# TUM-DAML/gemnet_pytorch

Hardware: AMD Instinct MI355X
Metric: molecules/sec (forward+force) GemNet-T on COLL-shaped batches (higher is better)
Workload: dtype f32

## Files before the change

gemnet_pytorch_amd/csrc/radial_head.hip:

```cpp
#include "common.h"
#include "basis_math.h"

namespace {

constexpr int RH_NR = 6, RH_S = 7, RH_NI = 16;
constexpr int RH_NFUN = RH_NR + RH_S * RH_NR;
constexpr int RH_NOUT = 3 + RH_S;

constexpr int RH_LPE = 16, RH_BLOCK = 256, RH_EPB = RH_BLOCK / RH_LPE;

__device__ __forceinline__ float rh_distance(const float* __restrict__ R, int c, int a, float& vx, float& vy, float& vz) {
  const float* Ra = R + 3 * (int64_t)a;
  const float* Rc = R + 3 * (int64_t)c;
  vx = Ra[0] - Rc[0]; vy = Ra[1] - Rc[1]; vz = Ra[2] - Rc[2];
  return sqrtf(vx * vx + vy * vy + vz * vz);
}

__global__ void __launch_bounds__(RH_BLOCK)
radial_head_fwd_kernel(const float* __restrict__ R, const int32_t* __restrict__ id_c, const int32_t* __restrict__ id_a,
                       const float* __restrict__ freq, const float* __restrict__ z, const double* __restrict__ nrm,
                       const float* __restrict__ wcat, float* __restrict__ rbf, float* __restrict__ rbf3,
                       float* __restrict__ rbf_h, float* __restrict__ rbf_out, float* __restrict__ rbf_W1, int64_t E,
                       double cutoff, int p) {
  __shared__ float vals[RH_EPB][RH_NFUN];
// ... 53 lines not shown
  const int64_t e = blockIdx.x * (int64_t)RH_EPB + el;
  const bool ok = e < E;
  float vx = 0.f, vy = 0.f, vz = 0.f, d = 1.f;
  double g = 0.0;
  if (ok) {
    d = rh_distance(R, id_c[e], id_a[e], vx, vy, vz);
    const bool any_rbf = g_rbf || g_rbf3 || g_rbf_h || g_rbf_out;
    for (int j = sub; j < RH_NFUN; j += RH_LPE) {
      if (j < RH_NR) {
        if (!any_rbf) continue;
        float c = g_rbf ? g_rbf[e * RH_NR + j] : 0.f;
        if (g_rbf3) c += rh_dot16(wcat + (0 * RH_NR + j) * RH_NI, g_rbf3 + e * RH_NI);
        if (g_rbf_h) c += rh_dot16(wcat + (1 * RH_NR + j) * RH_NI, g_rbf_h + e * RH_NI);
        if (g_rbf_out) c += rh_dot16(wcat + (2 * RH_NR + j) * RH_NI, g_rbf_out + e * RH_NI);
        g += (double)c * bessel_rbf_eval((double)d, (double)freq[j], cutoff, p, 1, 0);
      } else if (g_rbf_W1) {
        const int lr = j - RH_NR, s = lr / RH_NR;
        const float c = rh_dot16(wcat + (3 * RH_NR + lr) * RH_NI, g_rbf_W1 + (e * RH_S + s) * RH_NI);
        g += (double)c * sph_radial_eval((double)d, (double)z[lr], nrm[lr], s, cutoff, p, 1);
      }
    }
  }
  part[el][sub] = g;
  __syncthreads();
  if (ok && sub == 0) {
    double t = 0.0;
#pragma unroll
    for (int q = 0; q < RH_LPE; ++q) t += part[el][q];
    const float sc = (float)(t / (double)d);
    Wout[3 * e] = sc * vx; Wout[3 * e + 1] = sc * vy; Wout[3 * e + 2] = sc * vz;
  }
}

inline bool rh_aligned(const void* p) { return (reinterpret_cast<uintptr_t>(p) & 15u) == 0; }

inline bool rh_shape_ok(int64_t E, int NR, int S, int NI, int p) {
  return NR == RH_NR && S == RH_S && NI == RH_NI && p >= 2 && E < ((int64_t)1 << 34);
}

}

extern "C" int gn_radial_head_fwd_f32(const float* R, const int32_t* id_c, const int32_t* id_a, const float* freq,
                                      const float* z, const double* nrm, const float* wcat, float* rbf, float* rbf3,
                                      float* rbf_h, float* rbf_out, float* rbf_W1, int64_t E, int NR, int S, int NI,
                                      float cutoff, int p, void* stream) {
  if (E <= 0) return 0;
  if (!rh_shape_ok(E, NR, S, NI, p)) return (int)hipErrorInvalidValue;
  if (!R || !id_c || !id_a || !freq || !z || !nrm || !wcat || !rbf || !rbf3 || !rbf_h || !rbf_out || !rbf_W1)
    return (int)hipErrorInvalidValue;
  hipLaunchKernelGGL(radial_head_fwd_kernel, dim3((unsigned)((E + RH_EPB - 1) / RH_EPB)), dim3(RH_BLOCK), 0,
                     static_cast<hipStream_t>(stream), R, id_c, id_a, freq, z, nrm, wcat, rbf, rbf3, rbf_h, rbf_out, rbf_W1, E,
                     (double)cutoff, p);
  GN_LAUNCH_CHECK();
  return 0;
}

extern "C" int gn_radial_head_bwd_f32(const float* g_rbf, const float* g_rbf3, const float* g_rbf_h, const float* g_rbf_out,
                                      const float* g_rbf_W1, const float* R, const int32_t* id_c, const int32_t* id_a,
                                      const float* freq, const float* z, const double* nrm, const float* wcat, float* W,
                                      int64_t E, int NR, int S, int NI, float cutoff, int p, void* stream) {
  if (E <= 0) return 0;
  if (!rh_shape_ok(E, NR, S, NI, p)) return (int)hipErrorInvalidValue;
  if (!R || !id_c || !id_a || !freq || !z || !nrm || !wcat || !W) return (int)hipErrorInvalidValue;
  if (!rh_aligned(wcat) || !rh_aligned(g_rbf3) || !rh_aligned(g_rbf_h) || !rh_aligned(g_rbf_out) || !rh_aligned(g_rbf_W1))
    return (int)hipErrorInvalidValue;
  hipLaunchKernelGGL(radial_head_bwd_kernel, dim3((unsigned)((E + RH_EPB - 1) / RH_EPB)), dim3(RH_BLOCK), 0,
                     static_cast<hipStream_t>(stream), g_rbf, g_rbf3, g_rbf_h, g_rbf_out, g_rbf_W1, R, id_c, id_a, freq, z, nrm, wcat,
                     W, E, (double)cutoff, p);
  GN_LAUNCH_CHECK();
  return 0;
}
```

gemnet_pytorch_amd/kernels.py:

```python
import contextlib
import ctypes
import os
import threading

import torch

from . import _lib
from ._lib import (GN_ANG_F16, GN_CHAIN_MAX_OPS, GN_CHAIN_ROW, GN_SPLIT_F16X2_ROW, GemmArgs, addr, check, ptr,
                   require_device, stream)


def _f32c(t):
    if t.dtype != torch.float32:
        raise TypeError(f"HIP path is fp32; got {t.dtype}")
    return t.contiguous()


def _rowmajor(t):
    if t.dtype != torch.float32:
        raise TypeError(f"HIP path is fp32; got {t.dtype}")
    if t.dim() != 2:
        raise ValueError("2-D operand expected")
    if t.shape[0] > 0 and t.shape[1] > 0 and t.stride(1) == 1 and t.stride(0) >= t.shape[1]:
        return t
# ... 601 lines not shown
    if idx_c.shape != idx_a.shape or idx_c.dim() != 1 or idx_c.dtype != torch.int32 or idx_a.dtype != torch.int32:
        raise ValueError("radial head: id_c / id_a are (E,) int32")
    return _f32c(R), idx_c.contiguous(), idx_a.contiguous(), _f32c(freq), _f32c(z), nrm.contiguous(), _f32c(wcat)


def radial_head_fwd(R, idx_c, idx_a, freq, z, nrm, wcat, cutoff, p):
    R, idx_c, idx_a, freq, z, nrm, wcat = _radial_head_args(R, idx_c, idx_a, freq, z, nrm, wcat)
    E = idx_c.shape[0]
    NR, S, NI = RADIAL_HEAD_SHAPE
    new = lambda *shape: torch.empty(shape, device=R.device, dtype=torch.float32)
    rbf, rbf3, rbf_h, rbf_out, rbf_W1 = new(E, NR), new(E, NI), new(E, NI), new(E, NI), new(E, S, NI)
    check(_lib.load().gn_radial_head_fwd_f32(ptr(R), ptr(idx_c), ptr(idx_a), ptr(freq), ptr(z), ptr(nrm), ptr(wcat), ptr(rbf),
                                             ptr(rbf3), ptr(rbf_h), ptr(rbf_out), ptr(rbf_W1), E, NR, S, NI, cutoff, p,
                                             stream()), "gn_radial_head_fwd_f32")
    return rbf, rbf3, rbf_h, rbf_out, rbf_W1


def radial_head_bwd(g_rbf, g_rbf3, g_rbf_h, g_rbf_out, g_rbf_W1, R, idx_c, idx_a, freq, z, nrm, wcat, cutoff, p):
    R, idx_c, idx_a, freq, z, nrm, wcat = _radial_head_args(R, idx_c, idx_a, freq, z, nrm, wcat)
    E = idx_c.shape[0]
    NR, S, NI = RADIAL_HEAD_SHAPE
    gs = []
    for g, shape in ((g_rbf, (E, NR)), (g_rbf3, (E, NI)), (g_rbf_h, (E, NI)), (g_rbf_out, (E, NI)), (g_rbf_W1, (E, S, NI))):
        if g is not None:
            require_device(g)
            if tuple(g.shape) != shape:
                raise ValueError(f"radial head: cotangent of shape {tuple(g.shape)}, expected {shape}")
            g = _f32c(g)
        gs.append(g)
    W = torch.empty((E, 3), device=R.device, dtype=torch.float32)
    check(_lib.load().gn_radial_head_bwd_f32(*[ptr(g) for g in gs], ptr(R), ptr(idx_c), ptr(idx_a), ptr(freq), ptr(z), ptr(nrm),
                                             ptr(wcat), ptr(W), E, NR, S, NI, cutoff, p, stream()),
          "gn_radial_head_bwd_f32")
    return W


def trip_basis_fwd(R, tc, ta, tb, S, want_theta=False):
    require_device(R, tc, ta, tb)
    R = _f32c(R)
    T = tc.shape[0]
    Y = torch.empty((T, S), device=R.device, dtype=torch.float32)
    theta = torch.empty(T, device=R.device, dtype=torch.float32) if want_theta else None
    check(_lib.load().gn_trip_basis_fwd_f32(ptr(R), ptr(tc), ptr(ta), ptr(tb), ptr(Y), ptr(theta), T, S, stream()),
          "gn_trip_basis_fwd_f32")
    return Y, theta


def trip_basis_bwd(gY, R, tc, ta, tb):
    require_device(gY, R)
    gY, R = _f32c(gY), _f32c(R)
    T, S = gY.shape
    Gc = torch.empty((T, 3), device=R.device, dtype=torch.float32)
    Gb = torch.empty((T, 3), device=R.device, dtype=torch.float32)
    check(_lib.load().gn_trip_basis_bwd_f32(ptr(gY), ptr(R), ptr(tc), ptr(ta), ptr(tb), ptr(Gc), ptr(Gb), T, S,
                                            stream()), "gn_trip_basis_bwd_f32")
    return Gc, Gb


def dist_fwd(R, id_c, id_a):
    require_device(R, id_c, id_a)
    R = _f32c(R)
    D = torch.empty(id_c.shape[0], device=R.device, dtype=torch.float32)
    check(_lib.load().gn_dist_fwd_f32(ptr(R), ptr(id_c), ptr(id_a), ptr(D), id_c.shape[0], stream()), "gn_dist_fwd_f32")
    return D


# ... 933 lines not shown
```

gemnet_pytorch_amd/model/gemnet.py:

```python
import contextlib
import os

import torch

from .. import ops
from ..graph import GraphPlan
from .layers import (INV_SQRT_2, AtomEmbedding, BesselBasisLayer, Dense, EdgeEmbedding,
                     EfficientInteractionDownProjection, InteractionBlock,
                     InteractionBlockTripletsOnly, OutputBlock, SphericalBasisLayer, TensorBasisLayer)
from .scaling import AutomaticFit


_nullcontext = contextlib.nullcontext
_H3_GUARD = os.environ.get("GEMNET_H3_GUARD", "1") == "1"
_TRAIN_OVERLAP = os.environ.get("GEMNET_TRAIN_OVERLAP", "1") == "1"
_Q_OVERLAP = os.environ.get("GEMNET_Q_OVERLAP", "1") == "1"
_RBF_OUT_SIDE = os.environ.get("GEMNET_RBF_OUT_SIDE", "1") == "1"
_PLAN_LATE = os.environ.get("GEMNET_PLAN_LATE", "1") == "1"


def K_chain_mode():
    from .. import kernels
    return kernels.current_mode()

# ... 123 lines not shown

    @staticmethod
    def calculate_angles(R, plan):
        q = plan.quad_geom
        Ra = ops.gather_rows(R, q["a_of_exp"])
        Rb = ops.gather_rows(R, q["b_of_exp"])
        Rd = ops.gather_rows(R, q["d_of_exp"])
        R_ba, R_bd = Ra - Rb, Rd - Rb
        angle_abd = GemNet.calculate_neighbor_angles(R_ba, R_bd)
        R_bd_proj = ops.gather_rows(GemNet.vector_rejection(R_bd, R_ba), plan.quad.expand)

        Rc = ops.gather_rows(R, q["c_of_red"])
        Ra2 = ops.gather_rows(R, q["a_of_red"])
        Rb2 = ops.gather_rows(R, q["b_of_red"])
        R_ac, R_ab = Rc - Ra2, Rb2 - Ra2
        angle_cab = ops.gather_rows(GemNet.calculate_neighbor_angles(R_ab, R_ac)[:, None], q["reduce_cab"])[:, 0]
        R_ac_proj = ops.gather_rows(GemNet.vector_rejection(R_ac, R_ab), q["reduce_cab"])
        angle_cabd = GemNet.calculate_neighbor_angles(R_ac_proj, R_bd_proj)
        return angle_cab, angle_abd, angle_cabd

    def _energy(self, R, plan, V=None, force_terms=False, Vint=None):
        T = self.triplets_only
        b3 = self.cbf_basis3
        overlap = self.overlap_output_blocks and (not ops.train2_enabled() or _TRAIN_OVERLAP)
        side = self._side_stream(R.device) if overlap and R.is_cuda and (T or _Q_OVERLAP) else None
        fork = side is not None and ops.is_fused() and T
        main = torch.cuda.current_stream(R.device) if fork else None
        h = terms = rbf_W1_3 = rbf_h = rbf_out = None
        proj = (self.mlp_rbf3, self.mlp_rbf_h, self.mlp_rbf_out)
        head = (ops.is_fused() and T and V is None and not self.direct_forces and R.is_cuda
                and all(d.bias is None and not d.act for d in proj)
                and ops.radial_head_supported(tuple(d.weight for d in proj) + (self.mlp_cbf3.weight,), b3.z_ln,
                                              self.rbf_basis.frequencies))
        if ops.is_fused():
            if fork:
                side.wait_stream(main)
                with torch.cuda.stream(side):
                    sph3 = ops.share_gradient(self._trip_basis3(R, plan, V))
                    h = self.atom_emb(plan.z_rows)
                    terms = self.edge_emb.atom_terms(h)
                    ev_a = torch.cuda.Event()
                    ev_a.record(side)
            if V is not None:
                from .. import pbc
                D_ca, rbf, rad3 = pbc.edge_basis(V, self.rbf_basis.frequencies, b3.z_ln, b3.n_ln, b3.cutoff, b3.p)
                V_ca = None
            elif head:
                rbf, rbf3, rbf_h, rbf_out, rbf_W1_3 = self._radial_head(R, plan, proj)
                V_ca = None
            else:
                D_ca, V_ca, rbf, rad3 = ops.edge_basis(R, self.rbf_basis.frequencies, plan.id_c, plan.id_a,
                                                       b3.z_ln, b3.n_ln, b3.cutoff, b3.p,
                                                       want_V=self.direct_forces)
            if fork and head:
                main.wait_event(ev_a)
                for t in (sph3, h) + tuple(terms):
                    t.record_stream(main)
            elif fork:
                ev_1 = torch.cuda.Event()
                ev_1.record(main)
                side.wait_event(ev_1)
                with torch.cuda.stream(side):
                    rbf.record_stream(side)
                    rad3.record_stream(side)
                    rbf_W1_3 = self.mlp_cbf3(rad3)
                    rbf_h = self.mlp_rbf_h(rbf)
                    if _RBF_OUT_SIDE:
                        rbf_out = self.mlp_rbf_out(rbf)
                    ev_b = torch.cuda.Event()
                    ev_b.record(side)
                if not _RBF_OUT_SIDE:
                    rbf_out = self.mlp_rbf_out(rbf)
                main.wait_event(ev_a)
                for t in (sph3, h) + tuple(terms):
                    t.record_stream(main)
            else:
                sph3 = ops.share_gradient(self._trip_basis3(R, plan, V))
        elif ops.train2_enabled() and not self.direct_forces:
            from .. import ops_train
            if V is not None:
                D_ca, V_ca = ops_train.distances_vec(V), None
                angles = ops_train.triplet_angles_vec(V, plan.trip)
            else:
                D_ca, V_ca = ops_train.distances(R, plan.id_c, plan.id_a), None
                angles = ops_train.triplet_angles(R, plan.t_c, plan.t_a, plan.t_b)
            rbf = self.rbf_basis(D_ca)
            rad3, sph3 = b3(D_ca, angles)
        elif V is not None:
            D_ca, V_ca = torch.sqrt(torch.sum(V ** 2, dim=1)), None
# ... 20 lines not shown
            if self.mlp_cbf4.bias is None and not self.mlp_cbf4.act:
                cbf4 = ops.cbf_project(rad4, plan.intm_ab, y_abd, self.mlp_cbf4.weight)
            cbf4_done = cbf4 is not None
            if not cbf4_done:
                cbf4 = (ops.gather_rows(rad4, plan.intm_ab) * y_abd[:, :, None]).reshape(-1, S * NR)
            ang = self.int_blocks[0].quad_interaction.mlp_sbf.weight.shape[:2] == (32, 32)
            if V is not None:
                sbf4 = (rad3, ops.share_gradient(pbc.quad_basis(V, Vint, plan, S, angle_form=ang)))
            else:
                sbf4 = (rad3, ops.share_gradient(ops.quad_basis(R, plan.q_c, plan.q_a, plan.q_b, plan.q_d, S, plan=plan,
                                                                angle_form=ang)))
        elif not T:
            qi = self.int_blocks[0].quad_interaction.mlp_sbf.weight
            if (ops.train2_enabled() and not self.direct_forces and self.num_spherical == 7
                    and ops.quad_train2_enabled(qi.shape[0], qi.shape[1], self.num_spherical ** 2)):
                from .. import ops_train
                qg = plan.quad_geom
                D_ab = ops_train.distances(R, plan.int_b, plan.int_a)
                Phi_abd = ops_train.triplet_angles(R, qg["a_of_exp"], qg["b_of_exp"], qg["d_of_exp"])
                cbf4 = self.cbf_basis(D_ab, Phi_abd, plan.intm_ab)
                sbf4 = (rad3, ops_train.quad_angles(R, plan.q_c, plan.q_a, plan.q_b, plan.q_d, plan))
            else:
                if ops.train2_enabled() and not self.direct_forces:
                    from .. import ops_train
                    D_ab = ops_train.distances(R, plan.int_b, plan.int_a)
                else:
                    D_ab, _ = self.calculate_interatomic_vectors(R, plan.int_b, plan.int_a)
                Phi_cab, Phi_abd, Theta_cabd = self.calculate_angles(R, plan)
                cbf4 = self.cbf_basis(D_ab, Phi_abd, plan.intm_ab)
                sbf4 = (rad3, ops.ylm(Phi_cab, Theta_cabd, self.num_spherical))

        if h is None:
            h = self.atom_emb(plan.z_rows)
        rbf = ops.accumulate_gradient(rbf)
        m = self.edge_emb(h, rbf, plan.id_c, plan.id_a, terms=terms)

        if not T:
            rbf4 = ops.accumulate_gradient(self.mlp_rbf4(rbf))
            if not cbf4_done:
                cbf4 = self.mlp_cbf4(cbf4)
            cbf4 = ops.accumulate_gradient(cbf4)
            sbf4 = (ops.accumulate_gradient(self.mlp_sbf4(sbf4[0])), sbf4[1])
        else:
            rbf4 = cbf4 = sbf4 = None
        rbf3 = ops.accumulate_gradient(rbf3 if head else self.mlp_rbf3(rbf))
        if head:
            cbf3 = (ops.accumulate_gradient(rbf_W1_3), sph3)
            rbf_h = ops.accumulate_gradient(rbf_h)
        elif fork:
            main.wait_event(ev_b)
            for t in (rbf_W1_3, rbf_h):
                t.record_stream(main)
            cbf3 = (ops.accumulate_gradient(rbf_W1_3, stream=main), sph3)
            rbf_h = ops.accumulate_gradient(rbf_h, stream=main)
        else:
            cbf3 = (ops.accumulate_gradient(self.mlp_cbf3(rad3)), sph3)
            rbf_h = ops.accumulate_gradient(self.mlp_rbf_h(rbf))
            rbf_out = self.mlp_rbf_out(rbf)

        outs = []
        group = self._out_group_blocks(R, m, rbf_out)
        group_ms = []

        def ready():
            if side is None:
                return None
            ev = torch.cuda.Event()
            ev.record(torch.cuda.current_stream())
# ... 30 lines not shown
        else:
            E_a, F_ca = outs[-1][0], outs[0][1]
            if force_terms:
                F_ca = [F for _, F in outs]
                if side is not None:
                    for F in F_ca:
                        F.record_stream(torch.cuda.current_stream())
            else:
                for _, F in outs[1:]:
                    F_ca = F_ca + F

        E_mol = ops.segsum_rows(E_a, plan.batch_seg)
        if not self.extensive:
            E_mol = E_mol / plan.atoms_per_mol.clamp(min=1)[:, None]
        return E_mol, F_ca, V_ca

    def _out_group_blocks(self, R, m, rbf_out):
        if not (self.triplets_only and R.is_cuda and ops.is_fused() and ops.constant_weights() and not ops.train2_enabled()
                and not self.direct_forces and not AutomaticFit.fitting_mode and ops.USE_OUT_GROUP):
            return None
        blocks = []
        for ob in self.out_blocks:
            if not (ob.fuse_aggregate and not ob.direct_forces and ob.dense_rbf.bias is None and not ob.dense_rbf.act
                    and ob._stackable(ob.seq_energy) and ob.out_energy.bias is None and not ob.out_energy.act
                    and ob.out_energy.weight.shape[0] == 1):
                return None
            gemms = [ob.seq_energy[0].weight]
            for layer in ob.seq_energy[1:]:
                gemms += [layer.dense_mlp[0].weight, layer.dense_mlp[1].weight]
            blocks.append(dict(W_rbf=ob.dense_rbf.weight, scale=ob.scale_sum.scale_factor, gemms=gemms,
                               act0=bool(ob.seq_energy[0].act), w_out=ob.out_energy.weight))
        return blocks if ops.output_group_supported(blocks, [m] * len(blocks), rbf_out) else None

    def _radial_head(self, R, plan, proj):
        b3 = self.cbf_basis3
        return ops.radial_head(R, self.rbf_basis.frequencies, plan.id_c, plan.id_a, b3.z_ln, b3.n_ln,
                               tuple(d.weight for d in proj) + (self.mlp_cbf3.weight,), b3.cutoff, b3.p)

    def _trip_basis3(self, R, plan, V):
        if V is not None:
            from .. import pbc
            return pbc.trip_basis(V, plan.trip, self.num_spherical)
        return ops.trip_basis(R, plan.t_c, plan.t_a, plan.t_b, self.num_spherical)

    def forward(self, inputs, stress=False):
        periodic = inputs.get("cell") is not None
        if stress and not periodic:
            raise ValueError("stress=True needs a periodic batch (inputs['cell'])")
        if periodic and "cell_offsets" not in inputs:
            raise ValueError("a periodic batch needs its neighbour list with 'cell_offsets' (pbc.PeriodicGraphBuilder)")
        inputs = self.with_indices(inputs)
        with ops.exclusive():
            out = self._forward_guarded(inputs, stress)
        return out if (stress or not periodic) else out[:2]

    def with_indices(self, inputs):
        if "id_c" in inputs:
            return inputs
        from ..index_device import ensure_indices
        self._check_inputs(inputs["R"])
        if torch.cuda.is_current_stream_capturing():
            raise RuntimeError("inputs without index arrays inside a stream capture: call model.with_indices(inputs) first")
        cutoff, int_cutoff = self.cbf_basis3.cutoff, getattr(getattr(self, "cbf_basis", None), "cutoff", 10.0)
        if "cutoffs" in inputs:
            c = inputs["cutoffs"].detach().cpu().tolist()
            cutoff, int_cutoff = float(c[0]), float(c[1])
        return ensure_indices(inputs, cutoff, int_cutoff, self.triplets_only)

# ... 327 lines not shown
```

gemnet_pytorch_amd/ops.py:

```python
import contextlib

import os
import threading

import torch

from . import _lib
from . import kernels as K

_EXCLUSIVE = threading.RLock()


def exclusive():
    return _EXCLUSIVE


_PARAM_GRADS = True


@contextlib.contextmanager
def param_grads(enabled: bool):
    global _PARAM_GRADS
    old = _PARAM_GRADS
    _PARAM_GRADS = enabled
# ... 809 lines not shown
            and all(W.is_cuda and W.dtype == torch.float32 for W in weights))


def _radial_head_wcat(weights):
    key = ("rhead",) + tuple((W.data_ptr(), tuple(W.stride())) for W in weights)
    return _cached(key, tuple(W._version for W in weights), lambda: K.radial_head_weights(*[W.detach() for W in weights]))


class _RadialHead(torch.autograd.Function):

    @staticmethod
    def forward(ctx, R, freq, ri_c, ri_a, z, nrm, wcat, cutoff, p):
        outs = K.radial_head_fwd(R, ri_c.idx32, ri_a.idx32, freq, z, nrm, wcat, cutoff, p)
        ctx.save_for_backward(R, freq, z, nrm, wcat)
        ctx.cfg = (ri_c, ri_a, cutoff, p)
        ctx.set_materialize_grads(False)
        return outs

    @staticmethod
    @torch.autograd.function.once_differentiable
    def backward(ctx, g_rbf, g_rbf3, g_rbf_h, g_rbf_out, g_rbf_W1):
        R, freq, z, nrm, wcat = ctx.saved_tensors
        ri_c, ri_a, cutoff, p = ctx.cfg
        gR = None
        if ctx.needs_input_grad[0]:
            W = K.radial_head_bwd(g_rbf, g_rbf3, g_rbf_h, g_rbf_out, g_rbf_W1, R, ri_c.idx32, ri_a.idx32, freq, z, nrm, wcat,
                                  cutoff, p)
            gR = K.segsum_multi([(W, *ri_a.csr, 1.0), (W, *ri_c.csr, -1.0)], ri_a.n_rows)
        return gR, None, None, None, None, None, None, None, None


def radial_head(R, freq, ri_c, ri_a, z, nrm, weights, cutoff, p):
    return _RadialHead.apply(R, freq.detach(), ri_c, ri_a, z, nrm, _radial_head_wcat(weights), float(cutoff), int(p))


class _TripBasis(torch.autograd.Function):

    @staticmethod
    def forward(ctx, R, ri_c, ri_a, ri_b, S):
        Y, _ = K.trip_basis_fwd(R, ri_c.idx32, ri_a.idx32, ri_b.idx32, S)
        ctx.save_for_backward(R)
        ctx.cfg = (ri_c, ri_a, ri_b)
        return Y

    @staticmethod
    @torch.autograd.function.once_differentiable
    def backward(ctx, gY):
        (R,) = ctx.saved_tensors
        ri_c, ri_a, ri_b = ctx.cfg
        if not ctx.needs_input_grad[0]:
            return None, None, None, None, None
        Gc, Gb = K.trip_basis_bwd(gY, R, ri_c.idx32, ri_a.idx32, ri_b.idx32)
        gR = K.segsum_multi([(Gc, *ri_c.csr, 1.0), (Gb, *ri_b.csr, 1.0), (Gc, *ri_a.csr, -1.0), (Gb, *ri_a.csr, -1.0)],
                            ri_c.n_rows)
        return gR, None, None, None, None


def trip_basis(R, ri_c, ri_a, ri_b, S):
    return _TripBasis.apply(R, ri_c, ri_a, ri_b, int(S))


def constant_weights():
    return _FUSED and not _PARAM_GRADS


USE_STACKS = os.environ.get("GEMNET_STACKS", "1") == "1"
# ... 736 lines not shown
```

include/gemnet_hip.h:

```cpp
#ifndef GEMNET_HIP_H
#define GEMNET_HIP_H

#include <stdint.h>

#ifdef __cplusplus
extern "C" {
#endif

int gn_abi_version(void);
const char* gn_error_string(int code);

typedef struct {
  const float* A; const float* B; float* C;
  int M, N, K;
  int lda, ldb, ldc;
  int trans_a, trans_b;
  const float* a_dact_pre;
  int act;
  float* pre_out;
  const float* mul; int ldmul;
  float alpha;
  const float* res; int ldres;
  float beta;
  const float* gadd1; const int32_t* gidx1;
// ... 215 lines not shown
                         float* dSm, int64_t E, int S, int C, int I, int O, float alpha, int accumulate, void* stream);
int gn_bil_up_bwd_f32(const float* G, const int32_t* inv_swap, const float* z_ac, const float* z_ca, const void* Wupt_planes,
                      const void* W2_planes, const float* Sm, const float* B, float* gB, float* dSm, int64_t E, int S, int C, int I,
                      int O, int N_up, float alpha, float alpha_up, int act, int accumulate, void* stream);
int gn_bil_dy_multi_f32(const float* const* dSm_list, const float* const* x_list, int nb, const int32_t* expand_idx,
                        const int32_t* seg_off, float* dY, int64_t E, int S, int C, void* stream);
int gn_bil_dy_atoms_f32(const float* const* dSm_list, const float* const* x_list, int nb, const int32_t* grp_rows,
                        const int32_t* grp_off, const int32_t* ent_off, const int32_t* ent_t, const int32_t* ent_bc,
                        const int32_t* expand_idx, const int32_t* seg_off, float* dY, int64_t G, int max_rows, int S, int C,
                        void* stream);

int gn_bessel_rbf_f32(const float* d, const float* freq, float* out, int64_t E, int R,
                      float cutoff, int p, int kd, int kf, void* stream);
int gn_sph_radial_f32(const float* d, const float* z, const double* nrm, float* out, int64_t E,
                      int S, int R, float cutoff, int p, int kd, void* stream);
int gn_ylm0_f32(const float* theta, float* out, int64_t T, int S, int k, void* stream);
int gn_ylm_f32(const float* theta, const float* phi, float* out, int64_t Q, int S, int kt, int kp,
               void* stream);

int gn_edge_basis_fwd_f32(const float* R, const int32_t* id_c, const int32_t* id_a, const float* freq,
                          const float* z, const double* nrm, float* D, float* V, float* rbf, float* rad,
                          int64_t E, int NR, int S, float cutoff, int p, void* stream);
int gn_edge_basis_bwd_f32(const float* g_D, const float* g_rbf, const float* g_rad, const float* R,
                          const int32_t* id_c, const int32_t* id_a, const float* freq, const float* z,
                          const double* nrm, float* W, int64_t E, int NR, int S, float cutoff, int p,
                          void* stream);
int gn_radial_head_fwd_f32(const float* R, const int32_t* id_c, const int32_t* id_a, const float* freq, const float* z,
                           const double* nrm, const float* wcat, float* rbf, float* rbf3, float* rbf_h, float* rbf_out,
                           float* rbf_W1, int64_t E, int NR, int S, int NI, float cutoff, int p, void* stream);
int gn_radial_head_bwd_f32(const float* g_rbf, const float* g_rbf3, const float* g_rbf_h, const float* g_rbf_out,
                           const float* g_rbf_W1, const float* R, const int32_t* id_c, const int32_t* id_a,
                           const float* freq, const float* z, const double* nrm, const float* wcat, float* W, int64_t E,
                           int NR, int S, int NI, float cutoff, int p, void* stream);
int gn_trip_basis_fwd_f32(const float* R, const int32_t* tc, const int32_t* ta, const int32_t* tb, float* Y,
                          float* theta, int64_t T, int S, void* stream);
int gn_trip_basis_bwd_f32(const float* gY, const float* R, const int32_t* tc, const int32_t* ta,
                          const int32_t* tb, float* Gc, float* Gb, int64_t T, int S, void* stream);

int gn_dist_fwd_f32(const float* R, const int32_t* id_c, const int32_t* id_a, float* D, int64_t E, void* stream);
int gn_dist_bwd_f32(const float* gD, const float* R, const int32_t* id_c, const int32_t* id_a, float* W, int64_t E, void* stream);
int gn_dist_jvp_f32(const float* R, const float* tR, const float* gD, const int32_t* id_c, const int32_t* id_a, float* Ddot,
                    float* H, int64_t E, void* stream);
int gn_angle_fwd_f32(const float* R, const int32_t* tc, const int32_t* ta, const int32_t* tb, float* theta, int64_t T,
                     void* stream);
int gn_angle_bwd_f32(const float* g, const float* R, const int32_t* tc, const int32_t* ta, const int32_t* tb, float* Gc,
                     float* Gb, int64_t T, void* stream);
int gn_angle_jvp_f32(const float* R, const float* tR, const float* g, const int32_t* tc, const int32_t* ta, const int32_t* tb,
                     float* thdot, float* Hc, float* Hb, int64_t T, void* stream);

int gn_quad_basis_fwd_f32(const float* R, const int32_t* qc, const int32_t* qa, const int32_t* qb,
                          const int32_t* qd, float* Y, int64_t Q, int S, void* stream);
int gn_quad_basis_bwd_f32(const float* gY, const float* R, const int32_t* qc, const int32_t* qa,
                          const int32_t* qb, const int32_t* qd, float* Gc, float* Gb, float* Gd, int64_t Q,
                          int S, void* stream);
int gn_quad_basis_bwd_ld_f32(const float* gY, const float* R, const int32_t* qc, const int32_t* qa, const int32_t* qb,
                             const int32_t* qd, float* Gc, int ldc, float* Gb, int ldb, float* Gd, int ldd, int64_t Q,
                             int S, void* stream);

int gn_ssilu_f32(const float* x, float* out, int64_t n, int k, void* stream);
int gn_pm_f32(const float* z, int k, const float* a, const float* b, const float* d, float c, float* out,
              int64_t n, void* stream);
int gn_dact_mul_f32(const float* g, const float* z, int act, const float* mul, float c, float* dz,
                    float* gmul, int64_t n, void* stream);

int gn_optim_blocks(int64_t n);
int gn_adamw_ema_step_f32(float* p, const float* g, const float* gscale, const float* wd, float* m, float* v,
// ... 95 lines not shown
```

Baseline: 16860.

## Fuse edge embedding into radial head kernel using per-element atom term tables

Adds forward and backward radial-head kernels that also compute the edge embedding m = ssilu(T_c[z_c] + T_a[z_a] + rbf·W_r). They use precomputed per-element tables (embedding times weight slices), cached across calls by weight version. This removes the separate rbf materialisation, the atom-term gather and the dense GEMM over edges. The backward folds the embedding gradient into the rbf derivative path, which adds a 128-wide dot per rbf lane and extra stores of d0 in forward.

```diff
diff --git a/gemnet_pytorch_amd/csrc/radial_head.hip b/gemnet_pytorch_amd/csrc/radial_head.hip
--- a/gemnet_pytorch_amd/csrc/radial_head.hip
+++ b/gemnet_pytorch_amd/csrc/radial_head.hip
@@ -109,6 +109,144 @@
   }
 }
 
+constexpr int RH_NE = 128, RH_NE4 = RH_NE / 4;
+constexpr int RH_PITCH4 = RH_NE4 + 1;
+
+__global__ void __launch_bounds__(RH_BLOCK)
+radial_head_emb_fwd_kernel(const float* __restrict__ R, const int32_t* __restrict__ id_c, const int32_t* __restrict__ id_a,
+                           const float* __restrict__ freq, const float* __restrict__ z, const double* __restrict__ nrm,
+                           const float* __restrict__ wcat, const int32_t* __restrict__ zrow, const float4* __restrict__ Tc,
+                           const float4* __restrict__ Ta, const float4* __restrict__ Wr, float* __restrict__ rbf,
+                           float* __restrict__ rbf3, float* __restrict__ rbf_h, float* __restrict__ rbf_out,
+                           float* __restrict__ rbf_W1, float4* __restrict__ m0, float4* __restrict__ d0, int64_t E,
+                           double cutoff, int p) {
+  __shared__ float vals[RH_EPB][RH_NFUN];
+  __shared__ float4 wr[RH_NR * RH_NE4];
+  const int el = threadIdx.x / RH_LPE, sub = threadIdx.x % RH_LPE;
+  const int64_t e = blockIdx.x * (int64_t)RH_EPB + el;
+  const bool ok = e < E;
+  if (threadIdx.x < RH_NR * RH_NE4) wr[threadIdx.x] = Wr[threadIdx.x];
+  int c = 0, a = 0;
+  if (ok) {
+    float vx, vy, vz;
+    c = id_c[e]; a = id_a[e];
+    const float d = rh_distance(R, c, a, vx, vy, vz);
+    for (int j = sub; j < RH_NFUN; j += RH_LPE) {
+      float v;
+      if (j < RH_NR) {
+        v = (float)bessel_rbf_eval((double)d, (double)freq[j], cutoff, p, 0, 0);
+        if (rbf) rbf[e * RH_NR + j] = v;
+      } else {
+        const int lr = j - RH_NR;
+        v = (float)sph_radial_eval((double)d, (double)z[lr], nrm[lr], lr / RH_NR, cutoff, p, 0);
+      }
+      vals[el][j] = v;
+    }
+  }
+  __syncthreads();
+  if (!ok) return;
+  const int i = sub;
+#pragma unroll
+  for (int k = 0; k < RH_NOUT; ++k) {
+    const float* b = k < 3 ? vals[el] : vals[el] + RH_NR + (k - 3) * RH_NR;
+    const float* w = wcat + k * (RH_NR * RH_NI) + i;
+    float acc = b[0] * w[0];
+#pragma unroll
+    for (int r = 1; r < RH_NR; ++r) acc = fmaf(b[r], w[r * RH_NI], acc);
+    if (k >= 3) rbf_W1[(e * RH_S + (k - 3)) * RH_NI + i] = acc;
+    else (k == 0 ? rbf3 : (k == 1 ? rbf_h : rbf_out))[e * RH_NI + i] = acc;
+  }
+  const float4* tc = Tc + (int64_t)zrow[c] * RH_NE4;
+  const float4* ta = Ta + (int64_t)zrow[a] * RH_NE4;
+  const float* b = vals[el];
+#pragma unroll
+  for (int h = 0; h < 2; ++h) {
+    const int q = sub + h * RH_LPE;
+    const float4 g1 = tc[q], g2 = ta[q];
+    float4 v = make_float4(0.f, 0.f, 0.f, 0.f);
+#pragma unroll
+    for (int r = 0; r < RH_NR; ++r) {
+      const float4 w = wr[r * RH_NE4 + q];
+      v.x = fmaf(b[r], w.x, v.x); v.y = fmaf(b[r], w.y, v.y); v.z = fmaf(b[r], w.z, v.z); v.w = fmaf(b[r], w.w, v.w);
+    }
+    v.x += g1.x; v.y += g1.y; v.z += g1.z; v.w += g1.w;
+    v.x += g2.x; v.y += g2.y; v.z += g2.z; v.w += g2.w;
+    float4 dv;
+    gn_ssilu_pair(v.x, v.x, dv.x); gn_ssilu_pair(v.y, v.y, dv.y); gn_ssilu_pair(v.z, v.z, dv.z); gn_ssilu_pair(v.w, v.w, dv.w);
+    m0[e * RH_NE4 + q] = v;
+    d0[e * RH_NE4 + q] = dv;
+  }
+}
+
+__global__ void __launch_bounds__(RH_BLOCK)
+radial_head_emb_bwd_kernel(const float* __restrict__ g_rbf, const float* __restrict__ g_rbf3, const float* __restrict__ g_rbf_h,
+                           const float* __restrict__ g_rbf_out, const float* __restrict__ g_rbf_W1,
+                           const float4* __restrict__ ga, const float4* __restrict__ gb, const float4* __restrict__ d0,
+                           const float4* __restrict__ Wr, const float* __restrict__ R, const int32_t* __restrict__ id_c,
+                           const int32_t* __restrict__ id_a, const float* __restrict__ freq, const float* __restrict__ z,
+                           const double* __restrict__ nrm, const float* __restrict__ wcat, float* __restrict__ Wout, int64_t E,
+                           double cutoff, int p) {
+  __shared__ double part[RH_EPB][RH_LPE];
+  __shared__ float4 trow[RH_EPB][RH_PITCH4];
+  __shared__ float4 wr[RH_NR][RH_PITCH4];
+  const int el = threadIdx.x / RH_LPE, sub = threadIdx.x % RH_LPE;
+  const int64_t e = blockIdx.x * (int64_t)RH_EPB + el;
+  const bool ok = e < E;
+  const bool emb = ga || gb;
+  if (emb) {
+    if (threadIdx.x < RH_NR * RH_NE4) wr[threadIdx.x / RH_NE4][threadIdx.x % RH_NE4] = Wr[threadIdx.x];
+    if (ok) {
+#pragma unroll
+      for (int h = 0; h < 2; ++h) {
+        const int q = sub + h * RH_LPE;
+        float4 g = ga ? ga[e * RH_NE4 + q] : gb[e * RH_NE4 + q];
+        if (ga && gb) { const float4 u = gb[e * RH_NE4 + q]; g.x += u.x; g.y += u.y; g.z += u.z; g.w += u.w; }
+        const float4 dv = d0[e * RH_NE4 + q];
+        trow[el][q] = make_float4(g.x * dv.x, g.y * dv.y, g.z * dv.z, g.w * dv.w);
+      }
+    }
+    __syncthreads();
+  }
+  float vx = 0.f, vy = 0.f, vz = 0.f, d = 1.f;
+  double g = 0.0;
+  if (ok) {
+    d = rh_distance(R, id_c[e], id_a[e], vx, vy, vz);
+    const bool any_rbf = g_rbf || g_rbf3 || g_rbf_h || g_rbf_out || emb;
+    for (int j = sub; j < RH_NFUN; j += RH_LPE) {
+      if (j < RH_NR) {
+        if (!any_rbf) continue;
+        float c = g_rbf ? g_rbf[e * RH_NR + j] : 0.f;
+        if (g_rbf3) c += rh_dot16(wcat + (0 * RH_NR + j) * RH_NI, g_rbf3 + e * RH_NI);
+        if (g_rbf_h) c += rh_dot16(wcat + (1 * RH_NR + j) * RH_NI, g_rbf_h + e * RH_NI);
+        if (g_rbf_out) c += rh_dot16(wcat + (2 * RH_NR + j) * RH_NI, g_rbf_out + e * RH_NI);
+        if (emb) {
+          float s = 0.f;
+#pragma unroll 8
+          for (int q = 0; q < RH_NE4; ++q) {
+            const float4 t = trow[el][q], w = wr[j][q];
+            s = fmaf(t.x, w.x, s); s = fmaf(t.y, w.y, s); s = fmaf(t.z, w.z, s); s = fmaf(t.w, w.w, s);
+          }
+          c += s;
+        }
+        g += (double)c * bessel_rbf_eval((double)d, (double)freq[j], cutoff, p, 1, 0);
+      } else if (g_rbf_W1) {
+        const int lr = j - RH_NR, s = lr / RH_NR;
+        const float c = rh_dot16(wcat + (3 * RH_NR + lr) * RH_NI, g_rbf_W1 + (e * RH_S + s) * RH_NI);
+        g += (double)c * sph_radial_eval((double)d, (double)z[lr], nrm[lr], s, cutoff, p, 1);
+      }
+    }
+  }
+  part[el][sub] = g;
+  __syncthreads();
+  if (ok && sub == 0) {
+    double t = 0.0;
+#pragma unroll
+    for (int q = 0; q < RH_LPE; ++q) t += part[el][q];
+    const float sc = (float)(t / (double)d);
+    Wout[3 * e] = sc * vx; Wout[3 * e + 1] = sc * vy; Wout[3 * e + 2] = sc * vz;
+  }
+}
+
 inline bool rh_aligned(const void* p) { return (reinterpret_cast<uintptr_t>(p) & 15u) == 0; }
 
 inline bool rh_shape_ok(int64_t E, int NR, int S, int NI, int p) {
@@ -128,6 +266,48 @@
   hipLaunchKernelGGL(radial_head_fwd_kernel, dim3((unsigned)((E + RH_EPB - 1) / RH_EPB)), dim3(RH_BLOCK), 0,
                      static_cast<hipStream_t>(stream), R, id_c, id_a, freq, z, nrm, wcat, rbf, rbf3, rbf_h, rbf_out, rbf_W1, E,
                      (double)cutoff, p);
+  GN_LAUNCH_CHECK();
+  return 0;
+}
+
+extern "C" int gn_radial_head_emb_fwd_f32(const float* R, const int32_t* id_c, const int32_t* id_a, const float* freq,
+                                          const float* z, const double* nrm, const float* wcat, const int32_t* zrow,
+                                          const float* Tc, const float* Ta, const float* Wr, float* rbf, float* rbf3,
+                                          float* rbf_h, float* rbf_out, float* rbf_W1, float* m0, float* d0, int64_t E,
+                                          int NR, int S, int NI, int NE, float cutoff, int p, void* stream) {
+  if (E <= 0) return 0;
+  if (!rh_shape_ok(E, NR, S, NI, p) || NE != RH_NE) return (int)hipErrorInvalidValue;
+  if (!R || !id_c || !id_a || !freq || !z || !nrm || !wcat || !zrow || !Tc || !Ta || !Wr || !rbf3 || !rbf_h || !rbf_out ||
+      !rbf_W1 || !m0 || !d0)
+    return (int)hipErrorInvalidValue;
+  if (!rh_aligned(Tc) || !rh_aligned(Ta) || !rh_aligned(Wr) || !rh_aligned(m0) || !rh_aligned(d0))
+    return (int)hipErrorInvalidValue;
+  hipLaunchKernelGGL(radial_head_emb_fwd_kernel, dim3((unsigned)((E + RH_EPB - 1) / RH_EPB)), dim3(RH_BLOCK), 0,
+                     static_cast<hipStream_t>(stream), R, id_c, id_a, freq, z, nrm, wcat, zrow,
+                     reinterpret_cast<const float4*>(Tc), reinterpret_cast<const float4*>(Ta),
+                     reinterpret_cast<const float4*>(Wr), rbf, rbf3, rbf_h, rbf_out, rbf_W1, reinterpret_cast<float4*>(m0),
+                     reinterpret_cast<float4*>(d0), E, (double)cutoff, p);
+  GN_LAUNCH_CHECK();
+  return 0;
+}
+
+extern "C" int gn_radial_head_emb_bwd_f32(const float* g_rbf, const float* g_rbf3, const float* g_rbf_h, const float* g_rbf_out,
+                                          const float* g_rbf_W1, const float* ga, const float* gb, const float* d0,
+                                          const float* Wr, const float* R, const int32_t* id_c, const int32_t* id_a,
+                                          const float* freq, const float* z, const double* nrm, const float* wcat, float* W,
+                                          int64_t E, int NR, int S, int NI, int NE, float cutoff, int p, void* stream) {
+  if (E <= 0) return 0;
+  if (!rh_shape_ok(E, NR, S, NI, p) || NE != RH_NE) return (int)hipErrorInvalidValue;
+  if (!R || !id_c || !id_a || !freq || !z || !nrm || !wcat || !W) return (int)hipErrorInvalidValue;
+  if ((ga || gb) && (!d0 || !Wr)) return (int)hipErrorInvalidValue;
+  if (!rh_aligned(wcat) || !rh_aligned(g_rbf3) || !rh_aligned(g_rbf_h) || !rh_aligned(g_rbf_out) || !rh_aligned(g_rbf_W1) ||
+      !rh_aligned(ga) || !rh_aligned(gb) || !rh_aligned(d0) || !rh_aligned(Wr))
+    return (int)hipErrorInvalidValue;
+  hipLaunchKernelGGL(radial_head_emb_bwd_kernel, dim3((unsigned)((E + RH_EPB - 1) / RH_EPB)), dim3(RH_BLOCK), 0,
+                     static_cast<hipStream_t>(stream), g_rbf, g_rbf3, g_rbf_h, g_rbf_out, g_rbf_W1,
+                     reinterpret_cast<const float4*>(ga), reinterpret_cast<const float4*>(gb),
+                     reinterpret_cast<const float4*>(d0), reinterpret_cast<const float4*>(Wr), R, id_c, id_a, freq, z, nrm, wcat,
+                     W, E, (double)cutoff, p);
   GN_LAUNCH_CHECK();
   return 0;
 }
diff --git a/gemnet_pytorch_amd/kernels.py b/gemnet_pytorch_amd/kernels.py
--- a/gemnet_pytorch_amd/kernels.py
+++ b/gemnet_pytorch_amd/kernels.py
@@ -657,6 +657,73 @@
     check(_lib.load().gn_radial_head_bwd_f32(*[ptr(g) for g in gs], ptr(R), ptr(idx_c), ptr(idx_a), ptr(freq), ptr(z), ptr(nrm),
                                              ptr(wcat), ptr(W), E, NR, S, NI, cutoff, p, stream()),
           "gn_radial_head_bwd_f32")
+    return W
+
+
+RADIAL_EMB_WIDTH = 128
+
+
+def _aligned16(*tensors):
+    for t in tensors:
+        if t is not None and t.data_ptr() % 16:
+            raise ValueError("radial head: the 128-column operands must be 16-byte aligned")
+
+
+def _radial_emb_args(E, n_atoms, zrow, T_c, T_a, W_r):
+    NR, NE = RADIAL_HEAD_SHAPE[0], RADIAL_EMB_WIDTH
+    if tuple(W_r.shape) != (NR, NE):
+        raise ValueError(f"radial head: W_r of shape {tuple(W_r.shape)}, expected {(NR, NE)} (the rbf columns, transposed)")
+    if zrow is not None:
+        if T_c.dim() != 2 or T_c.shape[1] != NE or T_a.shape != T_c.shape:
+            raise ValueError(f"radial head: atom-term tables {tuple(T_c.shape)} / {tuple(T_a.shape)}, expected two (rows, {NE})")
+        if zrow.dim() != 1 or zrow.dtype != torch.int32 or zrow.shape[0] < n_atoms:
+            raise ValueError("radial head: zrow is (atoms,) int32, one table row per atom")
+        T_c, T_a, zrow = _f32c(T_c), _f32c(T_a), zrow.contiguous()
+    W_r = _f32c(W_r)
+    _aligned16(T_c, T_a, W_r)
+    require_device(zrow, T_c, T_a, W_r)
+    return zrow, T_c, T_a, W_r
+
+
+def radial_head_emb_fwd(R, idx_c, idx_a, freq, z, nrm, wcat, zrow, T_c, T_a, W_r, cutoff, p, want_rbf=False):
+    E = idx_c.shape[0]
+    NR, S, NI = RADIAL_HEAD_SHAPE
+    NE = RADIAL_EMB_WIDTH
+    zrow, T_c, T_a, W_r = _radial_emb_args(E, R.shape[0], zrow, T_c, T_a, W_r)
+    R, idx_c, idx_a, freq, z, nrm, wcat = _radial_head_args(R, idx_c, idx_a, freq, z, nrm, wcat)
+    new = lambda *shape: torch.empty(shape, device=R.device, dtype=torch.float32)
+    rbf3, rbf_h, rbf_out, rbf_W1, m0, d0 = new(E, NI), new(E, NI), new(E, NI), new(E, S, NI), new(E, NE), new(E, NE)
+    rbf = new(E, NR) if want_rbf else None
+    check(_lib.load().gn_radial_head_emb_fwd_f32(ptr(R), ptr(idx_c), ptr(idx_a), ptr(freq), ptr(z), ptr(nrm), ptr(wcat),
+                                                 ptr(zrow), ptr(T_c), ptr(T_a), ptr(W_r), ptr(rbf), ptr(rbf3), ptr(rbf_h),
+                                                 ptr(rbf_out), ptr(rbf_W1), ptr(m0), ptr(d0), E, NR, S, NI, NE, cutoff, p,
+                                                 stream()), "gn_radial_head_emb_fwd_f32")
+    return m0, d0, rbf3, rbf_h, rbf_out, rbf_W1, rbf
+
+
+def radial_head_emb_bwd(g_rbf, g_rbf3, g_rbf_h, g_rbf_out, g_rbf_W1, ga, gb, d0, W_r, R, idx_c, idx_a, freq, z, nrm, wcat,
+                        cutoff, p):
+    E = idx_c.shape[0]
+    NR, S, NI = RADIAL_HEAD_SHAPE
+    NE = RADIAL_EMB_WIDTH
+    gs = []
+    for g, shape in ((g_rbf, (E, NR)), (g_rbf3, (E, NI)), (g_rbf_h, (E, NI)), (g_rbf_out, (E, NI)), (g_rbf_W1, (E, S, NI)),
+                     (ga, (E, NE)), (gb, (E, NE)), (d0, (E, NE))):
+        if g is not None:
+            if tuple(g.shape) != shape:
+                raise ValueError(f"radial head: cotangent of shape {tuple(g.shape)}, expected {shape}")
+            g = _f32c(g)
+        gs.append(g)
+    if (gs[5] is not None or gs[6] is not None) and gs[7] is None:
+        raise ValueError("radial head: a cotangent of m0 needs d0")
+    _aligned16(*gs[5:])
+    _, _, _, W_r = _radial_emb_args(E, R.shape[0], None, None, None, W_r)
+    require_device(*gs)
+    R, idx_c, idx_a, freq, z, nrm, wcat = _radial_head_args(R, idx_c, idx_a, freq, z, nrm, wcat)
+    W = torch.empty((E, 3), device=R.device, dtype=torch.float32)
+    check(_lib.load().gn_radial_head_emb_bwd_f32(*[ptr(g) for g in gs], ptr(W_r), ptr(R), ptr(idx_c), ptr(idx_a), ptr(freq),
+                                                 ptr(z), ptr(nrm), ptr(wcat), ptr(W), E, NR, S, NI, NE, cutoff, p, stream()),
+          "gn_radial_head_emb_bwd_f32")
     return W
 
 
diff --git a/gemnet_pytorch_amd/model/gemnet.py b/gemnet_pytorch_amd/model/gemnet.py
--- a/gemnet_pytorch_amd/model/gemnet.py
+++ b/gemnet_pytorch_amd/model/gemnet.py
@@ -179,19 +179,27 @@
                 and all(d.bias is None and not d.act for d in proj)
                 and ops.radial_head_supported(tuple(d.weight for d in proj) + (self.mlp_cbf3.weight,), b3.z_ln,
                                               self.rbf_basis.frequencies))
+        ee = self.edge_emb
+        emb = head and ops.radial_emb_supported(self.atom_emb.embeddings.weight, ee.dense.weight, ee.dense.act, ee.dense.bias,
+                                                ee.atom_features)
+        m = None
         if ops.is_fused():
             if fork:
                 side.wait_stream(main)
                 with torch.cuda.stream(side):
                     sph3 = ops.share_gradient(self._trip_basis3(R, plan, V))
                     h = self.atom_emb(plan.z_rows)
-                    terms = self.edge_emb.atom_terms(h)
+                    if not emb:
+                        terms = self.edge_emb.atom_terms(h)
                     ev_a = torch.cuda.Event()
                     ev_a.record(side)
             if V is not None:
                 from .. import pbc
                 D_ca, rbf, rad3 = pbc.edge_basis(V, self.rbf_basis.frequencies, b3.z_ln, b3.n_ln, b3.cutoff, b3.p)
                 V_ca = None
+            elif emb:
+                m, rbf3, rbf_h, rbf_out, rbf_W1_3 = self._radial_head(R, plan, proj, emb=True)
+                rbf = V_ca = None
             elif head:
                 rbf, rbf3, rbf_h, rbf_out, rbf_W1_3 = self._radial_head(R, plan, proj)
                 V_ca = None
@@ -201,7 +209,7 @@
                                                        want_V=self.direct_forces)
             if fork and head:
                 main.wait_event(ev_a)
-                for t in (sph3, h) + tuple(terms):
+                for t in (sph3, h) + tuple(terms or ()):
                     t.record_stream(main)
             elif fork:
                 ev_1 = torch.cuda.Event()
@@ -288,8 +296,9 @@
 
         if h is None:
             h = self.atom_emb(plan.z_rows)
-        rbf = ops.accumulate_gradient(rbf)
-        m = self.edge_emb(h, rbf, plan.id_c, plan.id_a, terms=terms)
+        if m is None:
+            rbf = ops.accumulate_gradient(rbf)
+            m = self.edge_emb(h, rbf, plan.id_c, plan.id_a, terms=terms)
 
         if not T:
             rbf4 = ops.accumulate_gradient(self.mlp_rbf4(rbf))
@@ -386,8 +395,12 @@
                                act0=bool(ob.seq_energy[0].act), w_out=ob.out_energy.weight))
         return blocks if ops.output_group_supported(blocks, [m] * len(blocks), rbf_out) else None
 
-    def _radial_head(self, R, plan, proj):
+    def _radial_head(self, R, plan, proj, emb=False):
         b3 = self.cbf_basis3
+        if emb:
+            return ops.radial_head_emb(R, self.rbf_basis.frequencies, plan.id_c, plan.id_a, b3.z_ln, b3.n_ln,
+                                       tuple(d.weight for d in proj) + (self.mlp_cbf3.weight,), b3.cutoff, b3.p, plan.z_rows,
+                                       self.atom_emb.embeddings.weight, self.edge_emb.dense.weight, self.edge_emb.atom_features)
         return ops.radial_head(R, self.rbf_basis.frequencies, plan.id_c, plan.id_a, b3.z_ln, b3.n_ln,
                                tuple(d.weight for d in proj) + (self.mlp_cbf3.weight,), b3.cutoff, b3.p)
 
diff --git a/gemnet_pytorch_amd/ops.py b/gemnet_pytorch_amd/ops.py
--- a/gemnet_pytorch_amd/ops.py
+++ b/gemnet_pytorch_amd/ops.py
@@ -865,6 +865,61 @@
 
 def radial_head(R, freq, ri_c, ri_a, z, nrm, weights, cutoff, p):
     return _RadialHead.apply(R, freq.detach(), ri_c, ri_a, z, nrm, _radial_head_wcat(weights), float(cutoff), int(p))
+
+
+USE_RADIAL_EMB = os.environ.get("GEMNET_RADIAL_EMB", "1") == "1"
+ATOM_TABLE_BUILDS = 0
+
+
+def radial_emb_supported(emb_weight, W, act, bias, atom_features):
+    NR, NE = K.RADIAL_HEAD_SHAPE[0], K.RADIAL_EMB_WIDTH
+    return (USE_RADIAL_EMB and bias is None and bool(act) and atom_features == NE and tuple(W.shape) == (NE, 2 * NE + NR)
+            and tuple(emb_weight.shape) == (93, NE) and W.is_cuda and emb_weight.is_cuda
+            and W.dtype == torch.float32 and emb_weight.dtype == torch.float32 and K.current_mode() != "f32")
+
+
+def _make_atom_tables(emb_weight, W, A):
+    global ATOM_TABLE_BUILDS
+    ATOM_TABLE_BUILDS += 1
+    emb, W = emb_weight.detach(), W.detach()
+    T_c = K.gemm(emb, W[:, :A].contiguous())
+    T_a = K.gemm(emb, W[:, A:2 * A].contiguous())
+    return T_c, T_a, W[:, 2 * A:].t().contiguous()
+
+
+def atom_term_tables(emb_weight, W, A):
+    key = ("atab",) + tuple((t.data_ptr(), tuple(t.shape), tuple(t.stride())) for t in (emb_weight, W))
+    return _cached(key, (emb_weight._version, W._version), lambda: _make_atom_tables(emb_weight, W, A))
+
+
+class _RadialHeadEmb(torch.autograd.Function):
+
+    @staticmethod
+    def forward(ctx, R, freq, ri_c, ri_a, z, nrm, wcat, zrow, T_c, T_a, W_r, cutoff, p):
+        m0, d0, rbf3, rbf_h, rbf_out, rbf_W1, _ = K.radial_head_emb_fwd(R, ri_c.idx32, ri_a.idx32, freq, z, nrm, wcat, zrow,
+                                                                        T_c, T_a, W_r, cutoff, p)
+        ctx.save_for_backward(R, freq, z, nrm, wcat, d0, W_r)
+        ctx.cfg = (ri_c, ri_a, cutoff, p)
+        ctx.set_materialize_grads(False)
+        return m0, rbf3, rbf_h, rbf_out, rbf_W1
+
+    @staticmethod
+    @torch.autograd.function.once_differentiable
+    def backward(ctx, g_m0, g_rbf3, g_rbf_h, g_rbf_out, g_rbf_W1):
+        R, freq, z, nrm, wcat, d0, W_r = ctx.saved_tensors
+        ri_c, ri_a, cutoff, p = ctx.cfg
+        gR = None
+        if ctx.needs_input_grad[0]:
+            W = K.radial_head_emb_bwd(None, g_rbf3, g_rbf_h, g_rbf_out, g_rbf_W1, g_m0, None, d0, W_r, R, ri_c.idx32,
+                                      ri_a.idx32, freq, z, nrm, wcat, cutoff, p)
+            gR = K.segsum_multi([(W, *ri_a.csr, 1.0), (W, *ri_c.csr, -1.0)], ri_a.n_rows)
+        return (gR,) + (None,) * 12
+
+
+def radial_head_emb(R, freq, ri_c, ri_a, z, nrm, weights, cutoff, p, z_rows, emb_weight, W_emb, atom_features):
+    T_c, T_a, W_r = atom_term_tables(emb_weight, W_emb, atom_features)
+    return _RadialHeadEmb.apply(R, freq.detach(), ri_c, ri_a, z, nrm, _radial_head_wcat(weights), z_rows.idx32, T_c, T_a, W_r,
+                                float(cutoff), int(p))
 
 
 class _TripBasis(torch.autograd.Function):
diff --git a/include/gemnet_hip.h b/include/gemnet_hip.h
--- a/include/gemnet_hip.h
+++ b/include/gemnet_hip.h
@@ -271,6 +271,16 @@
                            const float* g_rbf_W1, const float* R, const int32_t* id_c, const int32_t* id_a,
                            const float* freq, const float* z, const double* nrm, const float* wcat, float* W, int64_t E,
                            int NR, int S, int NI, float cutoff, int p, void* stream);
+int gn_radial_head_emb_fwd_f32(const float* R, const int32_t* id_c, const int32_t* id_a, const float* freq, const float* z,
+                               const double* nrm, const float* wcat, const int32_t* zrow, const float* Tc, const float* Ta,
+                               const float* Wr, float* rbf, float* rbf3, float* rbf_h, float* rbf_out, float* rbf_W1,
+                               float* m0, float* d0, int64_t E, int NR, int S, int NI, int NE, float cutoff, int p,
+                               void* stream);
+int gn_radial_head_emb_bwd_f32(const float* g_rbf, const float* g_rbf3, const float* g_rbf_h, const float* g_rbf_out,
+                               const float* g_rbf_W1, const float* ga, const float* gb, const float* d0, const float* Wr,
+                               const float* R, const int32_t* id_c, const int32_t* id_a, const float* freq, const float* z,
+                               const double* nrm, const float* wcat, float* W, int64_t E, int NR, int S, int NI, int NE,
+                               float cutoff, int p, void* stream);
 int gn_trip_basis_fwd_f32(const float* R, const int32_t* tc, const int32_t* ta, const int32_t* tb, float* Y,
                           float* theta, int64_t T, int S, void* stream);
 int gn_trip_basis_bwd_f32(const float* gY, const float* R, const int32_t* tc, const int32_t* ta,
```

Result: faster. 17080, median of 6 (+1.3%).
